# aras-p/UnityGaussianSplatting

Measured on AMD Instinct MI355X. Metric: Msplats/s rendered (sort+view+composite+resolve), bicycle-sized synthetic 6,131,954 splats, 1200x797, Medium; ms/frame in ms_per_step, higher is better.
Workload: dtype f32; 1 GPU; bicycle-sized synthetic 6,131,954 splats, 1200x797, Medium; sort_mode=visible_in_flight, frames_in_flight=2, frames_in_flight_impl=library, splats=6131954, views=1, views_per_rank=1, blend=exact, sort_nth_frame=1, tile_pairs_P=4376060, tile=32x16, visible_splats=1563698, parallelism=single GPU, rccl_ranks=0

## Files before the change

unitygaussiansplatting_amd/csrc/gs_api.hip:

```cpp
#include <stdarg.h>
#include <stdlib.h>

#include <atomic>
#include <new>
#include <utility>

#include "gs_common.h"

namespace gs {

static thread_local char g_err[512] = "";

void set_error_detail(const char* fmt, ...) {
    va_list ap;
    va_start(ap, fmt);
    vsnprintf(g_err, sizeof(g_err), fmt, ap);
    va_end(ap);
}
int32_t fail(int32_t code, const char* what) {
    set_error_detail("%s", what);
    return code;
}
int32_t fail_hip(hipError_t e, const char* what, const char* file, int line) {
    set_error_detail("%s failed: %s (%s:%d)", what, hipGetErrorString(e), file, line);
// ... 64 lines not shown
int32_t gs_context_create(int32_t device, void* hip_stream, gs_context** out) {
    if (!out) return fail(GS_ERR_INVALID_ARGUMENT, "out is null");
    *out = nullptr;
    int count = 0;
    if (hipGetDeviceCount(&count) != hipSuccess || count <= 0) return fail(GS_ERR_NO_DEVICE, "no HIP device visible");
    if (device < 0 || device >= count) return fail(GS_ERR_INVALID_ARGUMENT, "device index out of range");
    gs_context* ctx = new (std::nothrow) gs_context();
    if (!ctx) return fail(GS_ERR_OUT_OF_MEMORY, "host allocation");
    ctx->device = device;
    if (hipSetDevice(device) != hipSuccess) { delete ctx; return fail(GS_ERR_HIP, "hipSetDevice"); }
    if (hipGetDeviceProperties(&ctx->props, device) != hipSuccess) { delete ctx; return fail(GS_ERR_HIP, "hipGetDeviceProperties"); }
    ctx->cuCount = ctx->props.multiProcessorCount > 0 ? ctx->props.multiProcessorCount : 256;
    if (hip_stream) { ctx->stream = (hipStream_t)hip_stream; ctx->ownStream = false; }
    else {
        if (hipStreamCreateWithFlags(&ctx->stream, hipStreamNonBlocking) != hipSuccess) { delete ctx; return fail(GS_ERR_HIP, "hipStreamCreate"); }
        ctx->ownStream = true;
    }
    if (hipStreamCreateWithFlags(&ctx->aux, hipStreamNonBlocking) != hipSuccess) { gs_context_destroy(ctx); return fail(GS_ERR_HIP, "hipStreamCreate (aux)"); }
    if (ctx->evOrder.create(hipEventDisableTiming) != hipSuccess) { gs_context_destroy(ctx); return fail(GS_ERR_HIP, "hipEventCreate (evOrder)"); }
    const char* ov = getenv("GSPLAT_OVERLAP");
    ctx->overlap = ov && ov[0] == '1';
    const char* vg = getenv("GSPLAT_VIEW_GENERIC");
    ctx->viewGeneric = vg && vg[0] == '1';
    const char* sh = getenv("GSPLAT_SHARED_GPU");
    ctx->sharedGpu = (sh && (sh[0] == '0' || sh[0] == '1')) ? (sh[0] - '0') : -1;
    g_liveContexts[device % kMaxTrackedDevices].fetch_add(1, std::memory_order_relaxed);
    ctx->counted = true;
    *out = ctx;
    return GS_OK;
}

int32_t gs_context_destroy(gs_context* ctx) {
    if (!ctx) return GS_OK;
    (void)hipSetDevice(ctx->device);
    if (ctx->aux) { (void)hipStreamSynchronize(ctx->aux); (void)hipStreamDestroy(ctx->aux); }
    if (ctx->stream) (void)hipStreamSynchronize(ctx->stream);
    if (ctx->ownStream && ctx->stream) (void)hipStreamDestroy(ctx->stream);
    if (ctx->counted) g_liveContexts[ctx->device % kMaxTrackedDevices].fetch_sub(1, std::memory_order_relaxed);
    delete ctx;
    return GS_OK;
}

int32_t gs_context_synchronize(gs_context* ctx) {
    if (!ctx) return fail(GS_ERR_INVALID_ARGUMENT, "ctx is null");
    for (gs_context* c : ctx->children) GS_TRY(gs_context_synchronize(c));
    GS_TRY(bind_device(ctx));
// ... 135 lines not shown
        GS_HIP(hipStreamSynchronize(L->ctx->stream));
        L->visBaseIdentity = r->visBaseIdentity; L->visRankValid = false; L->visOrderValid = false;
        L->visHistDepth = r->visHistDepth;
        memcpy(L->visHist, r->visHist, sizeof(r->visHist));
        L->distancesStale = false;
    }
    return GS_OK;
}

int32_t gs_renderer_set_frames_in_flight(gs_renderer* r, int32_t frames) {
    if (!r || frames < 1 || frames > GS_MAX_FRAMES_IN_FLIGHT) return fail(GS_ERR_INVALID_ARGUMENT, "frames in flight must be in [1, GS_MAX_FRAMES_IN_FLIGHT]");
    if (r->laneOf) return fail(GS_ERR_INVALID_ARGUMENT, "a lane has no lanes of its own");
    const size_t want = frames > 1 ? (size_t)frames : 0u;
    if (r->lanes.size() == want) return GS_OK;
    GS_TRY(gs_context_synchronize(r->ctx));
    lanes_destroy(r);
    for (size_t k = 0; k < want; ++k) {
        gs_context* c = nullptr;
        gs_renderer* L = nullptr;
        int32_t rc = gs_context_create(r->ctx->device, nullptr, &c);
        if (rc == GS_OK) {
            c->internalLane = true;
            c->viewGeneric = r->ctx->viewGeneric;
            if (c->counted) { g_liveContexts[c->device % kMaxTrackedDevices].fetch_sub(1, std::memory_order_relaxed); c->counted = false; }
        }
        if (rc == GS_OK) rc = renderer_create_n(c, r->asset, r->n, &L);
        if (rc == GS_OK) L->laneOf = r;
        if (rc == GS_OK) {
            L->adaptTall = r->adaptTall;
            if (r->pairCapacity > L->pairCapacity) rc = gs_renderer_reserve_pairs(L, r->pairCapacity);
        }
        if (rc == GS_OK && r->cutoutCount) rc = gs_renderer_set_cutouts(L, (const gs_cutout*)r->cutoutsHost.get(), r->cutoutCount);
        if (rc != GS_OK) {
            if (L) (void)gs_renderer_destroy(L);
            if (c) (void)gs_context_destroy(c);
            lanes_destroy(r);
            return rc;
        }
        r->lanes.push_back(L);
        r->ctx->children.push_back(c);
    }
    if (r->deletedBits) {
        const int32_t rc = edit_deleted_to_lanes(r);
        if (rc != GS_OK) { lanes_destroy(r); return rc; }
    }
    {
// ... 733 lines not shown
```

unitygaussiansplatting_amd/csrc/gs_common.h:

```cpp
#pragma once
#include <hip/hip_runtime.h>
#include <hip/hip_ext.h>
#include <stdint.h>
#include <stdio.h>
#include <string.h>
#include <utility>
#include <vector>

#include "../../include/gsplat_c.h"
#include "gs_device_math.h"
#include "gs_handles.h"
#include "gs_params.h"

#ifdef GS_CHAIN_PRIO
#define GS_CHAIN_PRIORITY() __builtin_amdgcn_s_setprio(GS_CHAIN_PRIO)
#else
#define GS_CHAIN_PRIORITY() do { } while (0)
#endif
#ifdef GS_VIEW_PRIO
#define GS_VIEW_PRIORITY() __builtin_amdgcn_s_setprio(GS_VIEW_PRIO)
#else
#define GS_VIEW_PRIORITY() do { } while (0)
#endif

// ... 88 lines not shown
               TB_POSITION = 2 };

struct BinControl {
    unsigned long long pairCount;
    uint32_t pairCountClamped;
    uint32_t error;
    uint32_t tieLongRuns, tieLongest;
    uint32_t pad0[26];
    uint32_t visible;
    uint32_t pad1[31];
    uint32_t tickets[16 * 32];
};

}

struct gs_context {
    int device = 0;
    hipStream_t stream = nullptr;
    bool ownStream = false;
    hipStream_t aux = nullptr;
    bool overlap = false;
    gs::Event evOrder;
    bool viewGeneric = false;
    int sharedGpu = -1;
    bool counted = false;
    int cuCount = 0;
    hipDeviceProp_t props;
    std::vector<gs_context*> children;
    bool internalLane = false;
    bool sortBesideSiblings = false;
};
bool gs_shared_gpu(const gs_context* ctx);

struct gs_asset {
    gs_context* ctx = nullptr;
    gsm::AssetView view{};
    void* blobs[5] = {nullptr, nullptr, nullptr, nullptr, nullptr};
    gs::DevBuf<uint8_t> ownedBlobs[5];
    uint64_t sizes[5] = {0, 0, 0, 0, 0};
    bool owned = true;
};

struct gs_sorter {
    gs_context* ctx = nullptr;
    gs::SortState st;
    gs::DevBuf<gs::SortControl> control;
// ... 130 lines not shown
};

namespace gs {
inline int32_t signal_to(gs_context* from, hipStream_t waiter) {
    GS_HIP(order_after(waiter, from->stream, from->evOrder));
    return GS_OK;
}
inline gs_renderer* owner_of(gs_renderer* r) { return r->laneOf ? r->laneOf : r; }
inline const gs_renderer* owner_of(const gs_renderer* r) { return r->laneOf ? r->laneOf : r; }
void prof_record(gs_renderer* r, int k, hipStream_t st = nullptr);
int32_t target_touched(gs_target* t, hipStream_t st);
int32_t join_sort(gs_renderer* r);
int32_t mark_order_use(gs_renderer* r);
void prof_end_frame(gs_renderer* r);
int32_t sort_state_create(gs_context* ctx, SortState& st, uint32_t maxCount, bool smallPartitions = false);
int32_t enqueue_sort_keys(gs_context* ctx, hipStream_t st, const gsm::AssetView& a, const float* matSort, uint32_t* keyBySplat,
                          SortControl* control, SortControl* nextControl, uint32_t n, SortState& sort);
uint32_t sort_group_words(const SortState& st, uint32_t nUpper, int passes);
int32_t enqueue_histogram(gs_context* ctx, hipStream_t st, const uint32_t* keys, uint32_t n, const uint32_t* nPtr, int passes, uint32_t lastMask,
                          SortControl* control, SortState& sort);
int32_t enqueue_sort_passes(gs_context* ctx, hipStream_t stream, SortState& st, SortControl* control, uint32_t* keys, uint32_t* vals,
                            uint32_t nUpper, const uint32_t* nPtr, int passes, uint32_t lastMask = 255u,
                            gs_renderer* profR = nullptr, int evFirst = -1, int bitsPerPass = 8, const uint32_t* gatherKeys = nullptr, bool skipLastKeys = false,
                            uint32_t expected = 0);
int32_t enqueue_gather_keys(gs_context* ctx, const uint32_t* keyBySplat, const uint32_t* order, uint32_t* out, uint32_t n);
constexpr uint32_t kSortMaxCount = 1u << 30;
int32_t enqueue_set_indices(gs_context* ctx, uint32_t* order, uint32_t n);
inline bool vis_active(const gs_renderer* r) { return r->sortMode == GS_SORT_VISIBLE; }
int32_t vis_alloc(gs_renderer* r);
int32_t vis_push_matrix(gs_renderer* r, const float* matrixSort);
int32_t vis_consolidate(gs_renderer* r);
int32_t enqueue_tie_fix_full(gs_renderer* r, const uint32_t* keys, uint32_t* idx);
int32_t enqueue_visible_sort(gs_renderer* r);
inline const VisControl* vis_control(const gs_renderer* r) { return r->visControl + r->visControlIdx; }
int32_t enqueue_calc_view(gs_context* ctx, const gsm::AssetView& a, const gs_frame_params* p, const gsm::EditView& e, const ViewOutputs& out, bool full);
ViewOutputs view_outputs(gs_renderer* r);
int32_t renderer_alloc_raster(gs_renderer* r);
int32_t enqueue_draw(gs_renderer* r, const gs_frame_params* p, gs_target* rt);
void auto_tile_shape(uint32_t width, uint32_t height, uint32_t& wl, uint32_t& hl);
void pick_tile_shape(const gs_renderer* r, uint32_t width, uint32_t height, uint32_t& wl, uint32_t& hl);
int32_t enqueue_debug_points(gs_renderer* r, const gs_frame_params* p, gs_target* rt);
int32_t enqueue_debug_boxes(gs_renderer* r, const gs_frame_params* p, gs_target* rt, bool chunks);
int32_t enqueue_resolve(gs_target* t, const float bg[4], bool want8);
int32_t flush_clear(gs_target* t);
void edit_free(gs_renderer* r);
int32_t edit_ensure(gs_renderer* r);
int32_t edit_make_private(gs_renderer* r, int k);
// ... 57 lines not shown
```

unitygaussiansplatting_amd/csrc/gs_raster.hip:

```cpp
#include "gs_common.h"
#include <cstdlib>

namespace gs {

namespace {

struct RasterConsts {
    float W, H, nearClip, farClip;
    uint32_t tilesX, tilesY, width, height;
};

constexpr unsigned long long BFLAG_AGG = 1ull << 62, BFLAG_INCL = 2ull << 62, BVAL_MASK = (1ull << 62) - 1ull;
constexpr uint32_t BIN_SPIN_LIMIT = 1u << 24;

__device__ __forceinline__ float rl(float x, int b) { return __int_as_float(__builtin_amdgcn_readlane(__float_as_int(x), b)); }

__device__ __forceinline__ uint32_t wave_incl_scan_u32(uint32_t v) {
#define GS_DPP(x, ctrl, rowmask) (uint32_t)__builtin_amdgcn_update_dpp(0, (int)(x), ctrl, rowmask, 0xf, false)
    v += GS_DPP(v, 0x111, 0xf);
    v += GS_DPP(v, 0x112, 0xf);
    v += GS_DPP(v, 0x114, 0xf);
    v += GS_DPP(v, 0x118, 0xf);
    v += GS_DPP(v, 0x142, 0xa);
    v += GS_DPP(v, 0x143, 0xc);
// ... 46 lines not shown
    report->pairSortError = *pairSortError;
    report->tileShape = tileShape;
    report->tieLongRuns = binCtl->tieLongRuns; report->tieLongest = binCtl->tieLongest;
}

__device__ __forceinline__ uint32_t tile_bucket(uint32_t len, uint32_t lastCost) {
    if (len == 0) return 255u;
    const uint32_t pred = lastCost ? lastCost : min((len + 255u) >> 8, 12u) * 16u;
    return 254u - min(pred, 254u);
}
__device__ __forceinline__ uint32_t tile_cost_dilated(const uint32_t* tileCost, uint32_t t, uint32_t tilesX, uint32_t numTiles) {
    const uint32_t tilesY = numTiles / tilesX;
    const uint32_t y = t / tilesX, x = t - y * tilesX;
    const uint32_t x0 = x > 0u ? x - 1u : 0u, x1 = min(x + 1u, tilesX - 1u);
    const uint32_t y0 = y > 0u ? y - 1u : 0u, y1 = min(y + 1u, tilesY - 1u);
    const uint32_t r0 = y0 * tilesX, r1 = y * tilesX, r2 = y1 * tilesX;
    const uint32_t c[9] = { tileCost[r0 + x0], tileCost[r0 + x], tileCost[r0 + x1], tileCost[r1 + x0], tileCost[r1 + x], tileCost[r1 + x1],
                            tileCost[r2 + x0], tileCost[r2 + x], tileCost[r2 + x1] };
    uint32_t m = c[0];
#pragma unroll
    for (int i = 1; i < 9; ++i) m = max(m, c[i]);
    return m;
}
__device__ __forceinline__ void tile_order_body(const uint32_t* __restrict__ tileStart, const uint32_t* __restrict__ tileEnd,
                                                const uint32_t* tileCost, uint32_t numTiles, uint32_t tilesX, uint32_t* __restrict__ tileOrder,
                                                uint32_t* s_cnt, uint32_t* s_off, uint32_t* s_w, uint32_t nthreads) {
    auto bucket = [&](uint32_t t) -> uint32_t {
        const uint32_t c = tile_cost_dilated(tileCost, t, tilesX, numTiles);
        if (tileStart) return tile_bucket(tileEnd[t] - tileStart[t], c);
        return 254u - min(c, 254u);
    };
    const int tid = threadIdx.x, lane = tid & 63, w = tid >> 6;
    if (tid < 256) s_cnt[tid] = 0;
    __syncthreads();
    for (uint32_t t0 = tid; t0 < numTiles; t0 += 4u * nthreads) {
        uint32_t bk[4];
#pragma unroll
        for (int i = 0; i < 4; ++i) { const uint32_t t = t0 + (uint32_t)i * nthreads; bk[i] = t < numTiles ? bucket(t) : 0xffffffffu; }
#pragma unroll
        for (int i = 0; i < 4; ++i) if (bk[i] != 0xffffffffu) atomicAdd(&s_cnt[bk[i]], 1u);
    }
    __syncthreads();
    uint32_t v = 0, incl = 0;
    if (tid < 256) {
        v = s_cnt[tid];
        incl = v;
#pragma unroll
        for (int o = 1; o < 64; o <<= 1) { const uint32_t u = __shfl_up(incl, o, 64); if (lane >= o) incl += u; }
        if (lane == 63) s_w[w] = incl;
    }
    __syncthreads();
    if (tid < 256) {
// ... 510 lines not shown
    uint32_t* myHist = pairHist + (bid % histCopies) * (uint32_t)kHistStride;
    for (int j = tid; j < PASSES * 256; j += kEmitThreads) {
        const uint32_t c = s_hist[j];
        if (c) atomicAdd(&myHist[j], c);
    }
}

__global__ __launch_bounds__(256) void tile_ranges_kernel(const uint32_t* __restrict__ pairKeys, const uint32_t* nPtr,
                                                          uint32_t* __restrict__ tileStart, uint32_t* __restrict__ tileEnd, uint32_t numTiles) {
    GS_CHAIN_PRIORITY();
    const uint32_t n = *nPtr;
    const uint32_t octs = (n + 7u) >> 3;
    for (uint32_t q = blockIdx.x * 256u + threadIdx.x; q < octs; q += gridDim.x * 256u) {
        const uint32_t j0 = q << 3;
        const uint4 ka = ((const uint4*)pairKeys)[2u * q], kb = ((const uint4*)pairKeys)[2u * q + 1u];
        const uint32_t k[10] = { j0 ? pairKeys[j0 - 1u] : 0xffffffffu, ka.x, ka.y, ka.z, ka.w, kb.x, kb.y, kb.z, kb.w,
                                 (j0 + 8u < n) ? pairKeys[j0 + 8u] : 0xffffffffu };
#pragma unroll
        for (int c = 0; c < 8; ++c) {
            const uint32_t j = j0 + (uint32_t)c;
            if (j >= n) break;
            const uint32_t t = k[c + 1];
            if (t >= numTiles) continue;
            if (j == 0 || k[c] != t) tileStart[t] = j;
            if (j == n - 1 || k[c + 2] != t) tileEnd[t] = j + 1;
        }
    }
}

__device__ __forceinline__ float mix_mul_lo(uint32_t h, float x) {
    float d;
    asm("v_fma_mix_f32 %0, %1, %2, 0 op_sel_hi:[1,0,0]" : "=v"(d) : "v"(h), "v"(x));
    return d;
}
__device__ __forceinline__ float mix_mul_hi(uint32_t h, float x) {
    float d;
    asm("v_fma_mix_f32 %0, %1, %2, 0 op_sel:[1,0,0] op_sel_hi:[1,0,0]" : "=v"(d) : "v"(h), "v"(x));
    return d;
}
__device__ __forceinline__ float mix_mul_lo_sat_after_trans(uint32_t h, float x) {
    float d;
    asm("s_nop 0\n\tv_fma_mix_f32 %0, %1, %2, 0 op_sel_hi:[1,0,0] clamp" : "=v"(d) : "v"(h), "v"(x));
    return d;
}
__device__ __forceinline__ float mix_one_minus_hi(uint32_t h) {
    float d;
    asm("v_fma_mix_f32 %0, %1, -1.0, 1.0 op_sel:[1,0,0] op_sel_hi:[1,0,0]" : "=v"(d) : "v"(h));
// ... 65 lines not shown
    constexpr int TW = 1 << TWL, TH = 1 << THL;
    constexpr int NWX = TW / 8, NW = NWX * (TH / 8);
    constexpr int NT = 64 * NW;
    constexpr uint32_t SLOTS = 2048u * 256u / (uint32_t)NT;
    __shared__ float4 s_a[NT];
    __shared__ uint4 s_b[NT];
    __shared__ float4 s_e[NT];
    __shared__ int s_done;
    __shared__ uint32_t s_cost;
    uint32_t survWalked = 0;

    const int tid = threadIdx.x, lane = tid & 63, w = tid >> 6;
#ifdef GS_BLEND_TL
    const unsigned long long tl0 = wall_clock64();
#endif
    if (blockIdx.x == 0 && tid == 0) write_report(binCtl, pairSortError, report, (uint32_t)TWL | ((uint32_t)THL << 8));
    const uint32_t tile = tileOrder[blockIdx.x];
#ifndef GS_BLEND_NOPRIO
    if (blockIdx.x < SLOTS / 8u) __builtin_amdgcn_s_setprio(3);
    else if (blockIdx.x < 3u * SLOTS / 8u) __builtin_amdgcn_s_setprio(2);
    else if (blockIdx.x < 6u * SLOTS / 8u) __builtin_amdgcn_s_setprio(1);
#endif
    const uint32_t tx = tile % rc.tilesX, ty = tile / rc.tilesX;
    const uint32_t start = tileStart[tile], end = tileEnd[tile];
    const int qx0 = (int)tx * TW + (w % NWX) * 8, qy0 = (int)ty * TH + (w / NWX) * 8;
    const int px = qx0 + (lane & 7), py = qy0 + (lane >> 3);
    const bool inside = px < (int)rc.width && py < (int)rc.height;
    uint2* dst = (uint2*)(rt + ((size_t)py * rc.width + (size_t)px) * 4);
    if (start >= end) {
        if (threadIdx.x == 0) tileCost[tile] = 0;
#ifdef GS_BLEND_TL
        if (threadIdx.x == 0 && blockIdx.x < 8192u) { unsigned long long* q = g_blendTl + blockIdx.x * 8u; q[0] = tl0; q[1] = wall_clock64(); q[2] = 0; q[3] = 0; q[4] = 0; q[5] = tile; q[6] = 0; }
#endif
        if (dstIsZero && inside) *dst = make_uint2(0u, 0u);
        return;
    }
    uint32_t batchesWalked = 0;

    const float fx = (float)px + 0.5f, fy = (float)py + 0.5f;
    const gsm::F2 fxy = { fx, fy };
    const float qminx = (float)qx0 + 0.5f, qmaxx = (float)qx0 + 7.5f, qminy = (float)qy0 + 0.5f, qmaxy = (float)qy0 + 7.5f;

    PixelAcc<MODE> acc;
    float sceneZ = 0.0f;
    if (DEPTH) sceneZ = inside ? sceneDepth[(size_t)py * rc.width + (size_t)px] : 0.0f;
    acc.load((inside && !dstIsZero) ? *dst : make_uint2(0u, 0u));
    if (tid == 0) s_done = 0;
// ... 205 lines not shown
            rect.x = (uint32_t)x0 | ((uint32_t)y0 << 16);
            rect.y = (uint32_t)(x1 + 1) | ((uint32_t)(y1 + 1) << 16);
            uint4* rp = (uint4*)(recs + idx);
            const uint32_t* w32 = (const uint32_t*)&rec;
#pragma unroll
            for (int k = 0; k < 4; ++k) rp[k] = make_uint4(w32[4 * k], w32[4 * k + 1], w32[4 * k + 2], w32[4 * k + 3]);
        }
        rects[idx] = rect;
    }
    const unsigned long long vb = __ballot(visible);
    if ((threadIdx.x & 63u) == 0u && idx < count) visMask[idx >> 6] = vb;
    if ((threadIdx.x & 63u) == 0u && idx < count) waveFlags[idx >> 6] = vb != 0ull ? 1u : 0u;
}

template <int MODE, bool DEPTH>
__global__ __launch_bounds__(256) void blend_box_kernel(const uint32_t* __restrict__ pairVals, const uint32_t* __restrict__ tileStart,
                                                        const uint32_t* __restrict__ tileEnd, const uint32_t* __restrict__ tileOrder,
                                                        uint32_t* __restrict__ tileCost, const gsm::BoxRec* __restrict__ recs, uint16_t* __restrict__ rt,
                                                        RasterConsts rc, gsm::RayConsts ray, int dstIsZero, const float* __restrict__ sceneDepth) {
    __shared__ uint4 s_rec[64 * 4];
    const int tid = threadIdx.x;
    const uint32_t tile = tileOrder[blockIdx.x];
    const uint32_t tx = tile % rc.tilesX, ty = tile / rc.tilesX;
    const uint32_t start = tileStart[tile], end = tileEnd[tile];
    const int px = (int)tx * 16 + (tid & 15), py = (int)ty * 16 + (tid >> 4);
    const bool inside = px < (int)rc.width && py < (int)rc.height;
    uint2* dst = (uint2*)(rt + ((size_t)py * rc.width + (size_t)px) * 4);
    if (start >= end) {
        if (tid == 0) tileCost[tile] = 0;
        if (dstIsZero && inside) *dst = make_uint2(0u, 0u);
        return;
    }
    PixelAcc<MODE> acc;
    acc.load((inside && !dstIsZero) ? *dst : make_uint2(0u, 0u));
    float sceneZ = 0.0f;
    if (DEPTH) sceneZ = inside ? sceneDepth[(size_t)py * rc.width + (size_t)px] : 0.0f;
    float d[3];
    gsm::PixelRay(ray, px, py, d);
    uint32_t walked = 0;
    for (uint32_t bs = start; bs < end; bs += 64u) {
        __syncthreads();
        const uint32_t cnt = min(64u, end - bs);
        {
            const uint32_t rix = (uint32_t)tid >> 2;
            if (rix < cnt) s_rec[tid] = ((const uint4*)(recs + pairVals[bs + rix]))[tid & 3];
        }
        __syncthreads();
// ... 209 lines not shown
        const uint32_t lastVis = (r->hostReport && r->frameInFlight) ? *(volatile uint32_t*)&r->hostReport.get()->visible : 0u;
        const uint32_t gridFor = lastVis ? min(count, lastVis + lastVis / 8u + 4096u) : count;
        const uint32_t vcGrid = max(1u, min(div_up(gridFor, kVcBlock * (uint32_t)(kVcThreads / 64)), (uint32_t)ctx->cuCount * 8u));
        hipLaunchKernelGGL(vis_count_kernel, dim3(vcGrid), dim3(kVcThreads), 0, st, (const uint2*)r->rects, order, vis, count, shapeKey, binCtl, binStatus, binGroupAgg,
                           r->visPairOffset, r->visRectX, r->visRectY,
                           r->pairSort.groupAgg, sort_group_words(r->pairSort, cap, passes), (uint32_t*)nextArena, (uint32_t)(r->frameArenaBytes / 4));
        hipLaunchKernelGGL(vis_offsets_kernel, dim3(vcGrid), dim3(kVcThreads), 0, st, vis, count, cap, binCtl, (const unsigned long long*)binStatus, (const unsigned long long*)binGroupAgg,
                           r->visPairOffset, r->visChunkStart, capChunks);
        const uint32_t emitGrid = (uint32_t)ctx->cuCount * (tileCnt ? 4u : 5u);
        r->pairSort.histCopies = hist_copies((int)emitGrid);
        auto emitKernel = passes == 1 ? (tileCnt ? vis_emit_kernel<1, true> : vis_emit_kernel<1, false>)
                        : (passes == 2 ? (tileCnt ? vis_emit_kernel<2, true> : vis_emit_kernel<2, false>) : vis_emit_kernel<3, false>);
        hipLaunchKernelGGL(emitKernel, dim3(emitGrid + (schedInBin ? 1u : 0u)), dim3(kEmitThreads), 0, st, order, (const uint32_t*)r->visRectX, (const uint32_t*)r->visRectY,
                           (const uint32_t*)r->visPairOffset, (const uint32_t*)r->visChunkStart, vis, count, (const BinControl*)binCtl, rc.tilesX, shapeKey, r->pairKeys, r->pairVals,
                           pairCtl->hist, (uint32_t)bits, o.costRead, numTiles, schedInBin ? o.tileOrder : (uint32_t*)nullptr, r->pairSort.histCopies);
    } else
    hipLaunchKernelGGL(binKernel, dim3(binGrid + (schedInBin ? 1u : 0u)), dim3(binThreads), 0, st, r->rects, wave_flags_of(r->visMask, r->n), order, count, rc.tilesX, shapeKey, r->pairKeys,
                       r->pairVals, cap, binCtl, binStatus, binGroupAgg, binGroupBase, pairCtl->hist, r->pairSort.groupAgg, sort_group_words(r->pairSort, cap, passes), (uint32_t*)nextArena, (uint32_t)(r->frameArenaBytes / 4),
                       (uint32_t)bits | (gs_shared_gpu(ctx) ? 0u : 0x100u), o.costRead, numTiles, schedInBin ? o.tileOrder : (uint32_t*)nullptr, r->pairSort.histCopies);
    GS_TRY(mark_order_use(r));
    prof_record(r, 4);
    const unsigned long long lastPairs = r->hostReport ? *(volatile unsigned long long*)&r->hostReport.get()->pairCount : 0ull;
    const uint32_t expectPairs = (uint32_t)(lastPairs < (unsigned long long)cap ? lastPairs : (unsigned long long)cap);
    GS_TRY(enqueue_sort_passes(ctx, st, r->pairSort, pairCtl, r->pairKeys, r->pairVals, cap, &binCtl->pairCountClamped, passes, 255u, r, 12, bits, nullptr, false,
                               expectPairs ? expectPairs : 1u));
    hipLaunchKernelGGL(tile_ranges_kernel, dim3(max(1u, min(div_up(cap, 2048), (uint32_t)ctx->cuCount * 8u))), dim3(256), 0, st, r->pairKeys,
                       &binCtl->pairCountClamped, o.tileStart, o.tileEnd, numTiles);
    r->lastPairPasses = (uint32_t)passes;
    o.binCtl = binCtl; o.pairSortError = &pairCtl->error;
    if (!schedInBin)
        hipLaunchKernelGGL(tile_order_kernel, dim3(1), dim3(1024), 0, st, o.tileStart, o.tileEnd, o.costRead, numTiles, rc.tilesX, o.tileOrder, binCtl, &pairCtl->error,
                           r->hostReport.device(), shapeKey);
    prof_record(r, 5);
    o.dstIsZero = rt->clearPending ? 1 : 0;
    rt->clearPending = false;
    return GS_OK;
}
}

static int forced_tile_shape() {
    static const int forced = [] {
        const char* e = getenv("GSPLAT_TILE");
        if (!e) return 0;
        if (!strcmp(e, "16x16")) return 1;
        if (!strcmp(e, "32x16")) return 2;
        if (!strcmp(e, "32x32")) return 3;
        return 0;
    }();
    return forced;
}
// ... 203 lines not shown
```

unitygaussiansplatting_amd/csrc/gs_sort.hip:

```cpp
#include "gs_common.h"
#include <cstdlib>

namespace gs {

namespace {

constexpr int RADIX = 256;
constexpr int THREADS = 512;
constexpr int WAVES = THREADS / 64;
constexpr int KPT_A = 16, KPT_B = 20, KPT_C = 8;
constexpr int PART_A = THREADS * KPT_A, PART_B = THREADS * KPT_B, PART_C = THREADS * KPT_C;
constexpr int PART_MIN = PART_C;
constexpr uint32_t kBigSortKeys = 24u << 20;
constexpr uint32_t kSmallSortKeys = 7u << 19;
constexpr uint32_t SPIN_LIMIT = 1u << 24;
constexpr uint32_t TICKET_CLASSES = 16;
constexpr int GROUP = 32;

constexpr uint32_t COUNT_BITS = 14, EPOCH_MASK = (1u << 18) - 1u;
static_assert(PART_A < (1 << COUNT_BITS) && PART_B < (1 << COUNT_BITS), "a partition's digit count must fit the status word");
__device__ __forceinline__ uint32_t pack_status(uint32_t epoch, uint32_t count) { return (epoch << COUNT_BITS) | count; }
__device__ __forceinline__ uint32_t ld_status(const uint32_t* p) { return __hip_atomic_load(p, __ATOMIC_RELAXED, __HIP_MEMORY_SCOPE_AGENT); }
__device__ __forceinline__ unsigned long long ld_word64(const unsigned long long* p) { return __hip_atomic_load(p, __ATOMIC_RELAXED, __HIP_MEMORY_SCOPE_AGENT); }
__device__ __forceinline__ void st_word64(unsigned long long* p, unsigned long long v) { __hip_atomic_store(p, v, __ATOMIC_RELAXED, __HIP_MEMORY_SCOPE_AGENT); }
// ... 101 lines not shown
            }
            const uint32_t key = gsm::SortKeyOf(pos, m20, m21, m22, m23);
            keyBySplat[idx] = key;
            lds_hist_add(s_h, key & 255u);
            lds_hist_add(s_h + RADIX, (key >> 8) & 255u);
            lds_hist_add(s_h + 2 * RADIX, (key >> 16) & 255u);
            lds_hist_add(s_h + 3 * RADIX, key >> 24);
        }
        if (more) {
#pragma unroll
            for (uint32_t k = 0; k < ILP; ++k) cur[k] = nxt[k];
        }
    }
    __syncthreads();
    uint32_t* myHist = hist + (blockIdx.x % copies) * (uint32_t)kHistStride;
    for (int j = threadIdx.x; j < 4 * RADIX; j += 1024) {
        const uint32_t c = s_h[j];
        if (c) atomicAdd(&myHist[j], c);
    }
}

constexpr int kLookbackBatch = 16;
constexpr int kMinWavesA = 6;
template <int BITS, bool GATHER, int KPT>
__global__ __launch_bounds__(THREADS, KPT == KPT_B ? 4 : kMinWavesA) void onesweep_kernel(const uint32_t* __restrict__ keysIn, const uint32_t* __restrict__ valsIn,
                                                           uint32_t* __restrict__ keysOut, uint32_t* __restrict__ valsOut,
                                                           const uint32_t* __restrict__ hist, uint32_t* status,
                                                           unsigned long long* groupAgg, unsigned long long* groupIncl, uint32_t* ticket, uint32_t* error,
                                                           uint32_t nImm, const uint32_t* nPtr, uint32_t shift, uint32_t epoch, uint32_t digitMask, uint32_t histCopies, uint32_t gatherXcd) {
    GS_CHAIN_PRIORITY();
    constexpr int PART = THREADS * KPT;
    constexpr int RDX = 1 << BITS;
    constexpr int DW = (RDX + 63) / 64;
    __shared__ uint32_t s_hist[WAVES * RDX];
    __shared__ uint32_t s_lbase[RDX];
    __shared__ uint32_t s_gbase[RDX];
    __shared__ __attribute__((aligned(16))) uint32_t s_pub[RDX];
    __shared__ uint32_t s_buf[PART];
    __shared__ uint32_t s_wtot[DW];
    __shared__ uint32_t s_htot[DW];
    __shared__ uint32_t s_part;

    const int tid = threadIdx.x, lane = tid & 63, w = tid >> 6;
    const uint32_t n = nPtr ? min(*nPtr, nImm) : nImm;
    const uint32_t numParts = (n + PART - 1) / PART;
    constexpr uint32_t kXcdMaxBlock = KPT == KPT_A ? 96 : 64;
    const uint32_t xcdRounds = (numParts + 8u * kXcdMaxBlock - 1u) / (8u * kXcdMaxBlock);
    const uint32_t xcdBlock = max(1u, (numParts + 8u * max(xcdRounds, 1u) - 1u) / (8u * max(xcdRounds, 1u)));
    (void)xcdBlock;

    uint32_t histExcl = 0;
    bool digitLive = false;
// ... 191 lines not shown
                            exclPrefix += (uint32_t)incl[b];
                            consumed = b + 1;
                            done = true;
                        } else if ((uint32_t)(agg[b] >> 40) == (uint32_t)GROUP) {
                            exclPrefix += (uint32_t)agg[b];
                            consumed = b + 1;
                        }
                    }
                    j -= consumed;
                    if (!done && consumed == 0) {
                        if (++spins > SPIN_LIMIT) { atomicOr(error, 1u); done = true; }
                        __builtin_amdgcn_s_sleep(1);
                    }
                }
            }
            if ((part % GROUP) == (uint32_t)(GROUP - 1) && total > 0 && digitLive)
                st_word64(groupIncl + (size_t)(part / GROUP) * RADIX + tid, ((unsigned long long)epoch << 32) | (unsigned long long)(exclPrefix + total));
            s_gbase[tid] = histExcl + exclPrefix - lbase;
        }
        __syncthreads();
        uint32_t dpack[(KPT + 3) / 4];
#pragma unroll
        for (int k = 0; k < (KPT + 3) / 4; ++k) dpack[k] = 0;
#pragma unroll
        for (int k = 0; k < KPT; ++k) {
            const uint32_t j = (uint32_t)tid + (uint32_t)k * THREADS;
            if (j < valid) {
                const uint32_t kk = s_buf[j];
                const uint32_t d = (kk >> shift) & digitMask;
                if (keysOut) stg32(keysOut, s_gbase[d] + j, kk);
                dpack[k >> 2] |= d << (8 * (k & 3));
            }
        }
        __syncthreads();
#pragma unroll
        for (int k = 0; k < KPT; ++k) s_buf[pos[k]] = val[k];
        __syncthreads();
#pragma unroll
        for (int k = 0; k < KPT; ++k) {
            const uint32_t j = (uint32_t)tid + (uint32_t)k * THREADS;
            if (j < valid) stg32(valsOut, s_gbase[(dpack[k >> 2] >> (8 * (k & 3))) & 255u] + j, s_buf[j]);
        }
    }
}

__global__ void copy_pairs_kernel(const uint32_t* __restrict__ ks, const uint32_t* __restrict__ vs, uint32_t* __restrict__ kd,
                                  uint32_t* __restrict__ vd, uint32_t nImm, const uint32_t* nPtr) {
    const uint32_t n = nPtr ? min(*nPtr, nImm) : nImm;
    for (uint32_t i = blockIdx.x * blockDim.x + threadIdx.x; i < n; i += gridDim.x * blockDim.x) { kd[i] = ks[i]; vd[i] = vs[i]; }
}

inline uint32_t div_up(uint32_t a, uint32_t b) { return (a + b - 1) / b; }

}


int32_t sort_state_create(gs_context* ctx, SortState& out, uint32_t maxCount, bool smallPartitions) {
    if (maxCount > kSortMaxCount) return fail(GS_ERR_INVALID_ARGUMENT, "sort capacity above 2^30 keys");
    SortState st;
    st.maxCount = maxCount;
    st.partMin = smallPartitions ? (uint32_t)PART_MIN : (uint32_t)PART_A;
    st.maxParts = div_up(maxCount > 0 ? maxCount : 1, st.partMin);
    GS_HIP(st.altKeys.alloc(((size_t)maxCount + 16) * 4));
    GS_HIP(st.altVals.alloc(((size_t)maxCount + 16) * 4));
    GS_HIP(st.status.alloc((size_t)st.maxParts * RADIX * 4));
    GS_HIP(hipMemsetAsync(st.status, 0, (size_t)st.maxParts * RADIX * 4, ctx->stream));
    st.maxGroups = div_up(st.maxParts, (uint32_t)GROUP);
    GS_HIP(st.groupAgg.alloc((size_t)4 * st.maxGroups * RADIX * 8));
    GS_HIP(st.groupIncl.alloc((size_t)st.maxGroups * RADIX * 8));
    GS_HIP(hipMemsetAsync(st.groupIncl, 0, (size_t)st.maxGroups * RADIX * 8, ctx->stream));
    out = std::move(st);
    return GS_OK;
// ... 27 lines not shown
    const uint32_t chunks = div_up(n, 256u);
    const uint32_t grid = max(1u, min(div_up(chunks, 4u * kKeysIlp), (uint32_t)ctx->cuCount));
    st.histCopies = hist_copies((int)grid);
#define GS_LAUNCH_KEYS(F) hipLaunchKernelGGL(sort_keys_kernel<F>, dim3(grid), dim3(1024), 0, stream, a, m[8], m[9], m[10], m[11], keyBySplat, \
                                             control->hist, n, st.groupAgg, sort_group_words(st, n, 4), (uint32_t*)nextControl, st.histCopies)
    switch (a.posFmt) { case 0: GS_LAUNCH_KEYS(0); break; case 1: GS_LAUNCH_KEYS(1); break; case 2: GS_LAUNCH_KEYS(2); break; default: GS_LAUNCH_KEYS(3); break; }
#undef GS_LAUNCH_KEYS
    GS_HIP(hipGetLastError());
    return GS_OK;
}

int32_t enqueue_histogram(gs_context* ctx, hipStream_t stream, const uint32_t* keys, uint32_t n, const uint32_t* nPtr, int passes, uint32_t lastMask, SortControl* control,
                          SortState& st) {
    GS_HIP(hipMemsetAsync(control, 0, sizeof(SortControl), stream));
    const uint32_t grid = max(1u, min(div_up(n, 256), (uint32_t)ctx->cuCount * 4u));
    st.histCopies = hist_copies((int)grid);
    hipLaunchKernelGGL(histogram_kernel, dim3(grid), dim3(256), 0, stream, keys, n, nPtr, passes, lastMask, control->hist, st.groupAgg, sort_group_words(st, n, passes), st.histCopies);
    GS_HIP(hipGetLastError());
    return GS_OK;
}

int32_t enqueue_sort_passes(gs_context* ctx, hipStream_t stream, SortState& st, SortControl* control, uint32_t* keys, uint32_t* vals, uint32_t nUpper,
                            const uint32_t* nPtr, int passes, uint32_t lastMask, gs_renderer* profR, int evFirst, int bits, const uint32_t* gatherKeys,
                            bool skipLastKeys, uint32_t expected) {
    const uint32_t histCopies = min(max(st.histCopies, 1u), (uint32_t)kHistReplicas);
    if (passes < 1 || passes > 4) return fail(GS_ERR_INVALID_ARGUMENT, "sort passes");
    if (bits < 6 || bits > 8 || (gatherKeys && bits != 8)) return fail(GS_ERR_INVALID_ARGUMENT, "sort digit width");
    if (nUpper > st.maxCount) return fail(GS_ERR_INVALID_ARGUMENT, "sort count exceeds sorter capacity");
    if (nUpper == 0) return GS_OK;
    static const int forcedShape = [] { const char* e = getenv("GSPLAT_SORT_SHAPE");
                                        return !e ? 0 : (e[0] == 'a' || e[0] == 'A') ? 1 : (e[0] == 'b' || e[0] == 'B') ? 2 : (e[0] == 'c' || e[0] == 'C') ? 3 : 0; }();
    const uint32_t expect = min(expected ? expected : nUpper, nUpper);
    const bool canC = bits == 8 && !gatherKeys && st.partMin <= (uint32_t)PART_C;
    const bool shapeC = canC && (forcedShape ? forcedShape == 3 : expect <= kSmallSortKeys);
    const bool shapeB = !shapeC && (forcedShape ? forcedShape == 2 : expect > kBigSortKeys);
    const uint32_t parts = div_up(nUpper, shapeC ? (uint32_t)PART_C : shapeB ? (uint32_t)PART_B : (uint32_t)PART_A);
    const uint32_t capacity = max(((uint32_t)ctx->cuCount * (shapeB ? 2u : 3u) / TICKET_CLASSES) * TICKET_CLASSES, TICKET_CLASSES);
    const uint32_t grid = min(div_up(parts, TICKET_CLASSES) * TICKET_CLASSES, capacity);
    uint32_t *ks = keys, *vs = vals, *kd = st.altKeys, *vd = st.altVals;
    const uint32_t groups = div_up(div_up(nUpper, st.partMin), (uint32_t)GROUP);
    const uint32_t fullMask = (1u << bits) - 1u;
    if (profR && evFirst >= 0) prof_record(profR, evFirst, stream);
    for (int p = 0; p < passes; ++p) {
        uint32_t epoch = (++st.epoch) & EPOCH_MASK;
        if (epoch == 0) {
            GS_HIP(hipMemsetAsync(st.status, 0, (size_t)st.maxParts * RADIX * 4, stream));
            GS_HIP(hipMemsetAsync(st.groupIncl, 0, (size_t)st.maxGroups * RADIX * 8, stream));
            st.epoch = epoch = 1;
        }
        const uint32_t* hist = control->hist + RADIX * p;
        unsigned long long* agg = st.groupAgg + (size_t)p * groups * RADIX;
        const uint32_t mask = p == passes - 1 ? (lastMask & fullMask) : fullMask;
        const uint32_t shift = (uint32_t)(bits * p);
        uint32_t* kdst = (skipLastKeys && p == passes - 1) ? (uint32_t*)nullptr : kd;
        hipEvent_t evStart = nullptr, evStop = nullptr;
        if (profR && profR->profiling && settings(profR).kernelTiming && !profR->ev.empty() && evFirst >= 0) {
            const int kb = profR->profCur * kEvPerFrame + (evFirst == 10 ? 14 : 22) + 2 * p;
            evStart = profR->ev[kb]; evStop = profR->ev[kb + 1];
            profR->evValid[kb] = profR->evValid[kb + 1] = 1;
        }
#define GS_LAUNCH_ONESWEEP_K(B, G, KIN, K) \
        hipExtLaunchKernelGGL((onesweep_kernel<B, G, K>), dim3(grid), dim3(THREADS), 0, stream, evStart, evStop, 0, (const uint32_t*)(KIN), (const uint32_t*)vs, kdst, vd, \
                              (const uint32_t*)hist, st.status.get(), agg, st.groupIncl.get(), (uint32_t*)control->tickets[p], &control->error, nUpper, nPtr, shift, epoch, mask, histCopies, gs_shared_gpu(ctx) ? 0u : ((gatherKeys ? 1u : 0u) | 2u))
#define GS_LAUNCH_ONESWEEP(B, G, KIN) do { if (shapeB) GS_LAUNCH_ONESWEEP_K(B, G, KIN, KPT_B); else GS_LAUNCH_ONESWEEP_K(B, G, KIN, KPT_A); } while (0)
        if (p == 0 && gatherKeys) GS_LAUNCH_ONESWEEP(8, true, gatherKeys);
        else if (shapeC) GS_LAUNCH_ONESWEEP_K(8, false, ks, KPT_C);
        else if (bits == 8) GS_LAUNCH_ONESWEEP(8, false, ks);
        else if (bits == 7) GS_LAUNCH_ONESWEEP(7, false, ks);
        else GS_LAUNCH_ONESWEEP(6, false, ks);
#undef GS_LAUNCH_ONESWEEP
#undef GS_LAUNCH_ONESWEEP_K
        uint32_t* t = ks; ks = kd; kd = t;
        t = vs; vs = vd; vd = t;
    }
    if (profR && evFirst >= 0) prof_record(profR, evFirst + 1, stream);
    if (ks != keys) {
        hipLaunchKernelGGL(copy_pairs_kernel, dim3(max(1u, min(div_up(nUpper, 256), (uint32_t)ctx->cuCount * 8u))), dim3(256), 0,
                           stream, ks, vs, keys, vals, nUpper, nPtr);
    }
    GS_HIP(hipGetLastError());
    return GS_OK;
}

}
```

Before: 16370 Msplats/s.

## Fuse tile range extraction into the last pair-sort pass and skip final key writes

Measured after the change: 16640 Msplats/s, median of 6. 1.6% higher.

```diff
diff --git a/unitygaussiansplatting_amd/csrc/gs_api.hip b/unitygaussiansplatting_amd/csrc/gs_api.hip
--- a/unitygaussiansplatting_amd/csrc/gs_api.hip
+++ b/unitygaussiansplatting_amd/csrc/gs_api.hip
@@ -110,6 +110,8 @@
     ctx->overlap = ov && ov[0] == '1';
     const char* vg = getenv("GSPLAT_VIEW_GENERIC");
     ctx->viewGeneric = vg && vg[0] == '1';
+    const char* tr = getenv("GSPLAT_TILE_RANGES");
+    ctx->tileRangesKernel = tr && !strcmp(tr, "kernel");
     const char* sh = getenv("GSPLAT_SHARED_GPU");
     ctx->sharedGpu = (sh && (sh[0] == '0' || sh[0] == '1')) ? (sh[0] - '0') : -1;
     g_liveContexts[device % kMaxTrackedDevices].fetch_add(1, std::memory_order_relaxed);
@@ -291,6 +293,7 @@
         if (rc == GS_OK) {
             c->internalLane = true;
             c->viewGeneric = r->ctx->viewGeneric;
+            c->tileRangesKernel = r->ctx->tileRangesKernel;
             if (c->counted) { g_liveContexts[c->device % kMaxTrackedDevices].fetch_sub(1, std::memory_order_relaxed); c->counted = false; }
         }
         if (rc == GS_OK) rc = renderer_create_n(c, r->asset, r->n, &L);
diff --git a/unitygaussiansplatting_amd/csrc/gs_common.h b/unitygaussiansplatting_amd/csrc/gs_common.h
--- a/unitygaussiansplatting_amd/csrc/gs_common.h
+++ b/unitygaussiansplatting_amd/csrc/gs_common.h
@@ -134,6 +134,7 @@
     bool overlap = false;
     gs::Event evOrder;
     bool viewGeneric = false;
+    bool tileRangesKernel = false;
     int sharedGpu = -1;
     bool counted = false;
     int cuCount = 0;
@@ -310,7 +311,8 @@
 int32_t enqueue_sort_passes(gs_context* ctx, hipStream_t stream, SortState& st, SortControl* control, uint32_t* keys, uint32_t* vals,
                             uint32_t nUpper, const uint32_t* nPtr, int passes, uint32_t lastMask = 255u,
                             gs_renderer* profR = nullptr, int evFirst = -1, int bitsPerPass = 8, const uint32_t* gatherKeys = nullptr, bool skipLastKeys = false,
-                            uint32_t expected = 0);
+                            uint32_t expected = 0,
+                            uint32_t* tileStart = nullptr, uint32_t* tileEnd = nullptr, uint32_t numTiles = 0);
 int32_t enqueue_gather_keys(gs_context* ctx, const uint32_t* keyBySplat, const uint32_t* order, uint32_t* out, uint32_t n);
 constexpr uint32_t kSortMaxCount = 1u << 30;
 int32_t enqueue_set_indices(gs_context* ctx, uint32_t* order, uint32_t n);
diff --git a/unitygaussiansplatting_amd/csrc/gs_raster.hip b/unitygaussiansplatting_amd/csrc/gs_raster.hip
--- a/unitygaussiansplatting_amd/csrc/gs_raster.hip
+++ b/unitygaussiansplatting_amd/csrc/gs_raster.hip
@@ -92,12 +92,13 @@
     for (int i = 1; i < 9; ++i) m = max(m, c[i]);
     return m;
 }
+__device__ __forceinline__ uint32_t tile_list_start(uint32_t startWord, uint32_t end) { return min(~startWord, end); }
 __device__ __forceinline__ void tile_order_body(const uint32_t* __restrict__ tileStart, const uint32_t* __restrict__ tileEnd,
                                                 const uint32_t* tileCost, uint32_t numTiles, uint32_t tilesX, uint32_t* __restrict__ tileOrder,
                                                 uint32_t* s_cnt, uint32_t* s_off, uint32_t* s_w, uint32_t nthreads) {
     auto bucket = [&](uint32_t t) -> uint32_t {
         const uint32_t c = tile_cost_dilated(tileCost, t, tilesX, numTiles);
-        if (tileStart) return tile_bucket(tileEnd[t] - tileStart[t], c);
+        if (tileStart) { const uint32_t end = tileEnd[t]; return tile_bucket(end - tile_list_start(tileStart[t], end), c); }
         return 254u - min(c, 254u);
     };
     const int tid = threadIdx.x, lane = tid & 63, w = tid >> 6;
@@ -654,7 +655,7 @@
             if (j >= n) break;
             const uint32_t t = k[c + 1];
             if (t >= numTiles) continue;
-            if (j == 0 || k[c] != t) tileStart[t] = j;
+            if (j == 0 || k[c] != t) tileStart[t] = ~j;
             if (j == n - 1 || k[c + 2] != t) tileEnd[t] = j + 1;
         }
     }
@@ -766,7 +767,7 @@
     else if (blockIdx.x < 6u * SLOTS / 8u) __builtin_amdgcn_s_setprio(1);
 #endif
     const uint32_t tx = tile % rc.tilesX, ty = tile / rc.tilesX;
-    const uint32_t start = tileStart[tile], end = tileEnd[tile];
+    const uint32_t end = tileEnd[tile], start = tile_list_start(tileStart[tile], end);
     const int qx0 = (int)tx * TW + (w % NWX) * 8, qy0 = (int)ty * TH + (w / NWX) * 8;
     const int px = qx0 + (lane & 7), py = qy0 + (lane >> 3);
     const bool inside = px < (int)rc.width && py < (int)rc.height;
@@ -1018,7 +1019,7 @@
     const int tid = threadIdx.x;
     const uint32_t tile = tileOrder[blockIdx.x];
     const uint32_t tx = tile % rc.tilesX, ty = tile / rc.tilesX;
-    const uint32_t start = tileStart[tile], end = tileEnd[tile];
+    const uint32_t end = tileEnd[tile], start = tile_list_start(tileStart[tile], end);
     const int px = (int)tx * 16 + (tid & 15), py = (int)ty * 16 + (tid >> 4);
     const bool inside = px < (int)rc.width && py < (int)rc.height;
     uint2* dst = (uint2*)(rt + ((size_t)py * rc.width + (size_t)px) * 4);
@@ -1274,10 +1275,12 @@
     prof_record(r, 4);
     const unsigned long long lastPairs = r->hostReport ? *(volatile unsigned long long*)&r->hostReport.get()->pairCount : 0ull;
     const uint32_t expectPairs = (uint32_t)(lastPairs < (unsigned long long)cap ? lastPairs : (unsigned long long)cap);
+    const bool rangesKernel = ctx->tileRangesKernel;
     GS_TRY(enqueue_sort_passes(ctx, st, r->pairSort, pairCtl, r->pairKeys, r->pairVals, cap, &binCtl->pairCountClamped, passes, 255u, r, 12, bits, nullptr, false,
-                               expectPairs ? expectPairs : 1u));
-    hipLaunchKernelGGL(tile_ranges_kernel, dim3(max(1u, min(div_up(cap, 2048), (uint32_t)ctx->cuCount * 8u))), dim3(256), 0, st, r->pairKeys,
-                       &binCtl->pairCountClamped, o.tileStart, o.tileEnd, numTiles);
+                               expectPairs ? expectPairs : 1u, rangesKernel ? (uint32_t*)nullptr : o.tileStart, rangesKernel ? (uint32_t*)nullptr : o.tileEnd, numTiles));
+    if (rangesKernel)
+        hipLaunchKernelGGL(tile_ranges_kernel, dim3(max(1u, min(div_up(cap, 2048), (uint32_t)ctx->cuCount * 8u))), dim3(256), 0, st, r->pairKeys,
+                           &binCtl->pairCountClamped, o.tileStart, o.tileEnd, numTiles);
     r->lastPairPasses = (uint32_t)passes;
     o.binCtl = binCtl; o.pairSortError = &pairCtl->error;
     if (!schedInBin)
diff --git a/unitygaussiansplatting_amd/csrc/gs_sort.hip b/unitygaussiansplatting_amd/csrc/gs_sort.hip
--- a/unitygaussiansplatting_amd/csrc/gs_sort.hip
+++ b/unitygaussiansplatting_amd/csrc/gs_sort.hip
@@ -147,12 +147,13 @@
 
 constexpr int kLookbackBatch = 16;
 constexpr int kMinWavesA = 6;
-template <int BITS, bool GATHER, int KPT>
+template <int BITS, bool GATHER, int KPT, bool RANGES = false>
 __global__ __launch_bounds__(THREADS, KPT == KPT_B ? 4 : kMinWavesA) void onesweep_kernel(const uint32_t* __restrict__ keysIn, const uint32_t* __restrict__ valsIn,
                                                            uint32_t* __restrict__ keysOut, uint32_t* __restrict__ valsOut,
                                                            const uint32_t* __restrict__ hist, uint32_t* status,
                                                            unsigned long long* groupAgg, unsigned long long* groupIncl, uint32_t* ticket, uint32_t* error,
-                                                           uint32_t nImm, const uint32_t* nPtr, uint32_t shift, uint32_t epoch, uint32_t digitMask, uint32_t histCopies, uint32_t gatherXcd) {
+                                                           uint32_t nImm, const uint32_t* nPtr, uint32_t shift, uint32_t epoch, uint32_t digitMask, uint32_t histCopies, uint32_t gatherXcd,
+                                                           uint32_t* tileStart, uint32_t* tileEnd, uint32_t numTiles) {
     GS_CHAIN_PRIORITY();
     constexpr int PART = THREADS * KPT;
     constexpr int RDX = 1 << BITS;
@@ -390,6 +391,7 @@
         uint32_t dpack[(KPT + 3) / 4];
 #pragma unroll
         for (int k = 0; k < (KPT + 3) / 4; ++k) dpack[k] = 0;
+        uint32_t runMask = 0;
 #pragma unroll
         for (int k = 0; k < KPT; ++k) {
             const uint32_t j = (uint32_t)tid + (uint32_t)k * THREADS;
@@ -397,7 +399,24 @@
                 const uint32_t kk = s_buf[j];
                 const uint32_t d = (kk >> shift) & digitMask;
                 if (keysOut) stg32(keysOut, s_gbase[d] + j, kk);
+                if (RANGES) runMask |= (uint32_t)(j == 0u || s_buf[max(j, 1u) - 1u] != kk) << k;
                 dpack[k >> 2] |= d << (8 * (k & 3));
+            }
+        }
+        if (RANGES) {
+            while (runMask) {
+                const uint32_t j = (uint32_t)tid + (uint32_t)(__ffs((int)runMask) - 1) * THREADS;
+                runMask &= runMask - 1u;
+                const uint32_t kk = s_buf[j];
+                if (kk < numTiles) __hip_atomic_fetch_max(tileStart + kk, ~(s_gbase[(kk >> shift) & digitMask] + j), __ATOMIC_RELAXED, __HIP_MEMORY_SCOPE_AGENT);
+                if (j) {
+                    const uint32_t pv = s_buf[j - 1u];
+                    if (pv < numTiles) __hip_atomic_fetch_max(tileEnd + pv, s_gbase[(pv >> shift) & digitMask] + j, __ATOMIC_RELAXED, __HIP_MEMORY_SCOPE_AGENT);
+                }
+            }
+            if (tid == 0 && valid) {
+                const uint32_t kk = s_buf[valid - 1u];
+                if (kk < numTiles) __hip_atomic_fetch_max(tileEnd + kk, s_gbase[(kk >> shift) & digitMask] + valid, __ATOMIC_RELAXED, __HIP_MEMORY_SCOPE_AGENT);
             }
         }
         __syncthreads();
@@ -415,7 +434,7 @@
 __global__ void copy_pairs_kernel(const uint32_t* __restrict__ ks, const uint32_t* __restrict__ vs, uint32_t* __restrict__ kd,
                                   uint32_t* __restrict__ vd, uint32_t nImm, const uint32_t* nPtr) {
     const uint32_t n = nPtr ? min(*nPtr, nImm) : nImm;
-    for (uint32_t i = blockIdx.x * blockDim.x + threadIdx.x; i < n; i += gridDim.x * blockDim.x) { kd[i] = ks[i]; vd[i] = vs[i]; }
+    for (uint32_t i = blockIdx.x * blockDim.x + threadIdx.x; i < n; i += gridDim.x * blockDim.x) { if (kd) kd[i] = ks[i]; vd[i] = vs[i]; }
 }
 
 inline uint32_t div_up(uint32_t a, uint32_t b) { return (a + b - 1) / b; }
@@ -489,11 +508,13 @@
 
 int32_t enqueue_sort_passes(gs_context* ctx, hipStream_t stream, SortState& st, SortControl* control, uint32_t* keys, uint32_t* vals, uint32_t nUpper,
                             const uint32_t* nPtr, int passes, uint32_t lastMask, gs_renderer* profR, int evFirst, int bits, const uint32_t* gatherKeys,
-                            bool skipLastKeys, uint32_t expected) {
+                            bool skipLastKeys, uint32_t expected, uint32_t* tileStart, uint32_t* tileEnd, uint32_t numTiles) {
     const uint32_t histCopies = min(max(st.histCopies, 1u), (uint32_t)kHistReplicas);
     if (passes < 1 || passes > 4) return fail(GS_ERR_INVALID_ARGUMENT, "sort passes");
     if (bits < 6 || bits > 8 || (gatherKeys && bits != 8)) return fail(GS_ERR_INVALID_ARGUMENT, "sort digit width");
     if (nUpper > st.maxCount) return fail(GS_ERR_INVALID_ARGUMENT, "sort count exceeds sorter capacity");
+    const bool ranges = tileStart != nullptr;
+    if (ranges && (!tileEnd || gatherKeys)) return fail(GS_ERR_INVALID_ARGUMENT, "sort tile ranges");
     if (nUpper == 0) return GS_OK;
     static const int forcedShape = [] { const char* e = getenv("GSPLAT_SORT_SHAPE");
                                         return !e ? 0 : (e[0] == 'a' || e[0] == 'A') ? 1 : (e[0] == 'b' || e[0] == 'B') ? 2 : (e[0] == 'c' || e[0] == 'C') ? 3 : 0; }();
@@ -519,31 +540,38 @@
         unsigned long long* agg = st.groupAgg + (size_t)p * groups * RADIX;
         const uint32_t mask = p == passes - 1 ? (lastMask & fullMask) : fullMask;
         const uint32_t shift = (uint32_t)(bits * p);
-        uint32_t* kdst = (skipLastKeys && p == passes - 1) ? (uint32_t*)nullptr : kd;
+        const bool rangesPass = ranges && p == passes - 1;
+        uint32_t* kdst = ((skipLastKeys || ranges) && p == passes - 1) ? (uint32_t*)nullptr : kd;
         hipEvent_t evStart = nullptr, evStop = nullptr;
         if (profR && profR->profiling && settings(profR).kernelTiming && !profR->ev.empty() && evFirst >= 0) {
             const int kb = profR->profCur * kEvPerFrame + (evFirst == 10 ? 14 : 22) + 2 * p;
             evStart = profR->ev[kb]; evStop = profR->ev[kb + 1];
             profR->evValid[kb] = profR->evValid[kb + 1] = 1;
         }
-#define GS_LAUNCH_ONESWEEP_K(B, G, KIN, K) \
-        hipExtLaunchKernelGGL((onesweep_kernel<B, G, K>), dim3(grid), dim3(THREADS), 0, stream, evStart, evStop, 0, (const uint32_t*)(KIN), (const uint32_t*)vs, kdst, vd, \
-                              (const uint32_t*)hist, st.status.get(), agg, st.groupIncl.get(), (uint32_t*)control->tickets[p], &control->error, nUpper, nPtr, shift, epoch, mask, histCopies, gs_shared_gpu(ctx) ? 0u : ((gatherKeys ? 1u : 0u) | 2u))
+#define GS_LAUNCH_ONESWEEP_KR(B, G, KIN, K, R) \
+        hipExtLaunchKernelGGL((onesweep_kernel<B, G, K, R>), dim3(grid), dim3(THREADS), 0, stream, evStart, evStop, 0, (const uint32_t*)(KIN), (const uint32_t*)vs, kdst, vd, \
+                              (const uint32_t*)hist, st.status.get(), agg, st.groupIncl.get(), (uint32_t*)control->tickets[p], &control->error, nUpper, nPtr, shift, epoch, mask, histCopies, gs_shared_gpu(ctx) ? 0u : ((gatherKeys ? 1u : 0u) | 2u), \
+                              tileStart, tileEnd, numTiles)
+#define GS_LAUNCH_ONESWEEP_K(B, G, KIN, K) GS_LAUNCH_ONESWEEP_KR(B, G, KIN, K, false)
 #define GS_LAUNCH_ONESWEEP(B, G, KIN) do { if (shapeB) GS_LAUNCH_ONESWEEP_K(B, G, KIN, KPT_B); else GS_LAUNCH_ONESWEEP_K(B, G, KIN, KPT_A); } while (0)
-        if (p == 0 && gatherKeys) GS_LAUNCH_ONESWEEP(8, true, gatherKeys);
+#define GS_LAUNCH_RANGES(B) do { if (shapeB) GS_LAUNCH_ONESWEEP_KR(B, false, ks, KPT_B, true); else GS_LAUNCH_ONESWEEP_KR(B, false, ks, KPT_A, true); } while (0)
+        if (rangesPass) { if (bits == 8) GS_LAUNCH_RANGES(8); else if (bits == 7) GS_LAUNCH_RANGES(7); else GS_LAUNCH_RANGES(6); }
+        else if (p == 0 && gatherKeys) GS_LAUNCH_ONESWEEP(8, true, gatherKeys);
         else if (shapeC) GS_LAUNCH_ONESWEEP_K(8, false, ks, KPT_C);
         else if (bits == 8) GS_LAUNCH_ONESWEEP(8, false, ks);
         else if (bits == 7) GS_LAUNCH_ONESWEEP(7, false, ks);
         else GS_LAUNCH_ONESWEEP(6, false, ks);
+#undef GS_LAUNCH_RANGES
 #undef GS_LAUNCH_ONESWEEP
 #undef GS_LAUNCH_ONESWEEP_K
+#undef GS_LAUNCH_ONESWEEP_KR
         uint32_t* t = ks; ks = kd; kd = t;
         t = vs; vs = vd; vd = t;
     }
     if (profR && evFirst >= 0) prof_record(profR, evFirst + 1, stream);
     if (ks != keys) {
         hipLaunchKernelGGL(copy_pairs_kernel, dim3(max(1u, min(div_up(nUpper, 256), (uint32_t)ctx->cuCount * 8u))), dim3(256), 0,
-                           stream, ks, vs, keys, vals, nUpper, nPtr);
+                           stream, ks, vs, ranges ? (uint32_t*)nullptr : keys, vals, nUpper, nPtr);
     }
     GS_HIP(hipGetLastError());
     return GS_OK;
```
